# LiuZhu-CV/PAIF

Hardware: AMD Instinct MI355X
Metric: fused image-pairs/sec at 480x640 bs=8 per GPU (fusion-net forward) (higher is better)
Workload: dtype f16 (IEEE fp16 maps and conv weights, one fp16 MFMA per product, f32 accumulate; stems, guided filter and the last map fp32)

## Files before the change

### paif_amd/csrc/conv_dma.h

```cpp
#pragma once
#include <hip/hip_runtime.h>

namespace paif_conv_dma {

struct Args {
  const void* src[3];
  const void* res[3];
  const void* wpk;
  const float* scale;
  const float* shift;
  const float* prelu;
  void* out;
  float alpha;
  int nsrc, nres, act, kh;
  int cout;
  int B, H, W, reverse;
  float* cpool;
  int f16;
  int dil;
  int in_relu;
};

bool eligible(int nsrc, int nres, int B, int H, int W, float alpha);
bool eligible16(int nsrc, int nres, int B, int H, int W, float alpha);
bool eligible7(int nsrc, int nres, int B, int H, int W, float alpha);
bool eligible_d2(int nsrc, int nres, int B, int H, int W, float alpha);
bool can_cpool(int nsrc, int nres, int kh, int cout, int dil);
int launch(const Args& a, hipStream_t st);

bool eligible_1x1(int nsrc, int nres, int B, int H, int W);
int launch_1x1(const Args& a, hipStream_t st);

}
```

### paif_amd/csrc/conv_mfma.hip

```cpp
#include <stdlib.h>

#include "conv_dma.h"
#include "paif_common.h"
#include <type_traits>

#ifndef PAIF_UB_HOOKS
#define PAIF_UB_HOOKS 3
#endif
#ifndef PAIF_UB
#define PAIF_UB 11
#endif

namespace {

typedef float f32x16 __attribute__((ext_vector_type(16)));

#ifndef PAIF_TH
#define PAIF_TH 8
#endif
constexpr int TH = PAIF_TH;
constexpr int TW = 32;
constexpr int NTHREADS = 256;
constexpr int SEGS_PER_WAVE = TH / 4;

// ... 1292 lines not shown
  } else {
    const int t = tid - 4 * 64;
    const int q = t & 7, px = t >> 3;
    const float4 sc = *reinterpret_cast<const float4*>((a.scale ? a.scale : k_ones) + 4 * q);
    const float4 sh = *reinterpret_cast<const float4*>((a.shift ? a.shift : k_zeros) + 4 * q);
    const float slope = *(a.act == 1 ? a.prelu : k_zeros);
    const int nres = a.res[0] ? (a.res[1] ? (a.res[2] ? 3 : 2) : 1) : 0;
    const unsigned lane_off = (unsigned)px * 32u + 4u * (unsigned)q;
    auto run = [&](auto nres_c) {
      constexpr int NR = decltype(nres_c)::value;
      float4 r[NR > 0 ? NR : 1][8];
      auto request = [&](int i) {
        int b, y0, x0;
        tile_of(min(i, cnt - 1), b, y0, x0);
        const size_t base = ((size_t)(b * a.H + y0) * a.W + x0) * 32;
        const unsigned lo = x0 + px < a.W ? lane_off : 0u;
#pragma unroll
        for (int k = 0; k < NR; ++k)
#pragma unroll
          for (int j = 0; j < 8; ++j) {
            const int yy = min(y0 + j, a.H - 1) - y0;
            r[k][j] = paif::ldq_nt<BFR>(a.res[k], base + (size_t)yy * a.W * 32 + lo);
          }
      };
      if (cnt > 0) request(0);
      int s2 = 0, i2 = 0;
      for (int g = 0; g <= S + 1; ++g) {
        if (g >= 2) {
          if (s2 == nsrc - 1) {
            int b, y0, x0;
            tile_of(i2, b, y0, x0);
            float4 o[8];
#pragma unroll
            for (int j = 0; j < 8; ++j) o[j] = *reinterpret_cast<const float4*>(outbuf + (j * 32 + px) * 32 + 4 * q);
            const size_t base = ((size_t)(b * a.H + y0) * a.W + x0) * 32;
            const bool colok = x0 + px < a.W;
#pragma unroll
            for (int j = 0; j < 8; ++j) {
              float4 v = o[j];
              v.x = v.x * sc.x + sh.x; v.y = v.y * sc.y + sh.y; v.z = v.z * sc.z + sh.z; v.w = v.w * sc.w + sh.w;
              if (a.act == 1) {
                v.x = paif::prelu_f(v.x, slope); v.y = paif::prelu_f(v.y, slope);
                v.z = paif::prelu_f(v.z, slope); v.w = paif::prelu_f(v.w, slope);
              } else if (a.act == 2) {
                v.x = fmaxf(v.x, 0.f); v.y = fmaxf(v.y, 0.f); v.z = fmaxf(v.z, 0.f); v.w = fmaxf(v.w, 0.f);
              }
              v.x *= a.alpha; v.y *= a.alpha; v.z *= a.alpha; v.w *= a.alpha;
#pragma unroll
              for (int k = 0; k < NR; ++k) { v.x += r[k][j].x; v.y += r[k][j].y; v.z += r[k][j].z; v.w += r[k][j].w; }
              if (colok && y0 + j < a.H)
                paif::stq_nt<BFO>(a.out, base + (size_t)j * a.W * 32 + lane_off, v);
              if (a.cpool) {
                float mx = fmaxf(fmaxf(v.x, v.y), fmaxf(v.z, v.w)), sm = (v.x + v.y) + (v.z + v.w);
                paif::pix8_max_sum(mx, sm);
                if (colok && y0 + j < a.H && q == 0)
                  *reinterpret_cast<float2*>(a.cpool + ((base + (size_t)j * a.W * 32) >> 5) * 4 + (size_t)px * 4) = make_float2(mx, sm * (1.0f / 32.0f));
              }
            }
            if (NR > 0) request(i2 + 1);
          }
          if (++s2 == nsrc) { s2 = 0; ++i2; }
        }
        lds_barrier();
        lds_barrier();
      }
    };
    if (nres == 0) run(std::integral_constant<int, 0>{});
    else if (nres == 1) run(std::integral_constant<int, 1>{});
    else if (nres == 2) run(std::integral_constant<int, 2>{});
    else run(std::integral_constant<int, 3>{});
  }
}

template <int KH, int DIL, int ST = 0>
__global__ __launch_bounds__(WS_THREADS, 1) void conv_bf16x3_ws(ConvArgs a, int ntiles) { conv_ws_body<KH, DIL, ST, false>(a, ntiles); }
template <int KH, int DIL, int ST = 0>
__global__ __launch_bounds__(WS_THREADS, 1) void conv_bf16x3_wsr(ConvArgs a, int ntiles) { conv_ws_body<KH, DIL, ST, true>(a, ntiles); }

template <int KH, int DIL, int ST = 0>
int launch_bf16x3_ws(const ConvArgs& a, hipStream_t st) {
  constexpr int P = DIL * (KH - 1) / 2;
  constexpr size_t lds_bytes = 2 * (size_t)(TH + 2 * P) * (TW + 2 * P) * 144 + 8 * 32 * 32 * 4;
  static_assert(lds_bytes <= 160 * 1024, "two tile buffers + the parked tile do not fit LDS");
  static bool raised = false;
  constexpr bool HAS_RELU = KH == 3 && DIL == 2 && paif::st_in(ST) != 0 && paif::st_low(ST) != 7;
  if (!raised) {
    hipError_t e = hipFuncSetAttribute(reinterpret_cast<const void*>(&conv_bf16x3_ws<KH, DIL, ST>),
                                       hipFuncAttributeMaxDynamicSharedMemorySize, (int)lds_bytes);
    if constexpr (HAS_RELU) {
      if (e == hipSuccess)
        e = hipFuncSetAttribute(reinterpret_cast<const void*>(&conv_bf16x3_wsr<KH, DIL, ST>), hipFuncAttributeMaxDynamicSharedMemorySize,
                                (int)lds_bytes);
    }
    if (e != hipSuccess) {
      paif::set_error("conv2d(bf16x3 ws): cannot raise dynamic LDS to %zu: %s", lds_bytes, hipGetErrorString(e));
      return (int)e;
    }
    raised = true;
  }
  if (a.in_act == 2) {
    if constexpr (HAS_RELU) {
      hipLaunchKernelGGL((conv_bf16x3_wsr<KH, DIL, ST>), dim3(256), dim3(WS_THREADS), lds_bytes, st, a, a.nblk);
      PAIF_LAUNCH_CHECK("conv2d(bf16x3 wsr)");
      return 0;
    }
    paif::set_error("conv2d(bf16x3 ws): input ReLU is built for the bf16-stored dilation-2 3x3 only");
    return PAIF_ENOSUP;
  }
  hipLaunchKernelGGL((conv_bf16x3_ws<KH, DIL, ST>), dim3(256), dim3(WS_THREADS), lds_bytes, st, a, a.nblk);
  PAIF_LAUNCH_CHECK("conv2d(bf16x3 ws)");
  return 0;
}

static inline bool ws_enabled() {
  static const bool on = [] {
    const char* e = getenv("PAIF_CONV_WS");
    return !(e && e[0] == '0');
  }();
  return on;
}
static inline bool st_h16(const ConvArgs& a) { return a.st == 1 || a.st == 3; }
static inline bool st_is_f16(const ConvArgs& a) { return a.st >= 3; }
static inline bool ws_eligible(const ConvArgs& a) {
  return ws_enabled() && a.nblk >= 1024 && !a.pool_partial && a.cout == 32 && (a.in_act == 0 || (a.in_act == 2 && st_h16(a))) &&
         (size_t)a.H * a.W * 128 < ((size_t)1 << 32);
}

static inline bool res_eligible(const ConvArgs& a) {
  static const bool on = [] {
    const char* e = getenv("PAIF_CONV_RES");
    return !(e && e[0] == '0');
  }();
  static const int ms_res = [] {
    const char* e = getenv("PAIF_CONV_RES_NSRC");
    return e ? atoi(e) : 1;
  }();
  return on && !st_is_f16(a) && (a.nsrc == 1 || (a.wl0 && a.st == 1 && a.in_act == 0 && a.nsrc <= ms_res)) && a.nblk >= 2048 && a.cout == 32 && a.in_act <= 2 && (PAIF_RES_ROWS == 8 || !a.pool_partial) &&
         (size_t)a.B * a.H * a.W * 128 < ((size_t)1 << 31);
}

static inline bool needs_hooks(const ConvArgs& a) { return a.in_act >= 3 || a.aux_out || a.epi_dact; }

static inline bool takes_ws(const ConvArgs& a, int kh, int dil) {
#if PAIF_TH == 8
  if (needs_hooks(a) || kh > 3 || !ws_eligible(a)) return false;
  if (a.st == 4) return dil == 2 && a.nsrc == 1 && a.in_act == 0;
  if (kh == 1) return !a.res[0] && a.in_act == 0;
  return dil == 2 && a.nsrc == 1 && st_h16(a);
#else
  return false;
#endif
}

enum ConvVariant { CV_PLAIN, CV_HOOKS, CV_WS, CV_RES, CV_MS, CV_DMA };
static inline int res_count(const ConvArgs& a) { return a.res[0] ? (a.res[1] ? (a.res[2] ? 3 : 2) : 1) : 0; }
static inline ConvVariant bf16x3_variant(const ConvArgs& a, int kh, int dil) {
  if (needs_hooks(a)) return CV_HOOKS;
  if (dil == 1 && st_h16(a) && a.wl0 && a.in_act == 0 && !a.pool_partial &&
      ((kh == 3 && a.cout == 32 && paif_conv_dma::eligible(a.nsrc, res_count(a), a.B, a.H, a.W, a.alpha)) ||
       (kh == 3 && a.cout == 16 && paif_conv_dma::eligible16(a.nsrc, res_count(a), a.B, a.H, a.W, a.alpha)) ||
       (kh == 7 && a.cout == 32 && paif_conv_dma::eligible7(a.nsrc, res_count(a), a.B, a.H, a.W, a.alpha))))
    return CV_DMA;
  if (kh == 3 && dil == 2 && st_h16(a) && a.wl0 && a.in_act == 2 && !a.pool_partial && a.cout == 32 &&
      paif_conv_dma::eligible_d2(a.nsrc, res_count(a), a.B, a.H, a.W, a.alpha))
    return CV_DMA;
  if (kh == 1 && dil == 1 && st_h16(a) && a.wl0 && a.in_act == 0 && !a.pool_partial && a.cout == 32 && ws_eligible(a) &&
      paif_conv_dma::eligible_1x1(a.nsrc, res_count(a), a.B, a.H, a.W))
    return CV_DMA;
  if (takes_ws(a, kh, dil)) return CV_WS;
  if (kh == 3 && dil == 1 && !st_is_f16(a)) {
    if (res_eligible(a)) return CV_RES;
    if (ms_enabled() && a.nsrc >= 2 && a.cout == 32 && a.in_act == 0 && !a.pool_partial &&
        (size_t)a.B * a.H * a.W * 128 < ((size_t)1 << 32))
      return CV_MS;
  }
  return CV_PLAIN;
}

static inline bool variant_can_cpool(const ConvArgs& a, int kh, int dil) {
  if (a.cout != 32 || needs_hooks(a)) return false;
  if (bf16x3_variant(a, kh, dil) == CV_DMA) return paif_conv_dma::can_cpool(a.nsrc, res_count(a), kh, a.cout, dil);
  return true;
}

template <int KH, int DIL, int ST>
int launch_bf16x3_st(const ConvArgs& a, hipStream_t st) {
  switch (bf16x3_variant(a, KH, DIL)) {
    case CV_DMA: {
      paif_conv_dma::Args d{};
      for (int s = 0; s < 3; ++s) { d.src[s] = a.src[s]; d.res[s] = a.res[s]; }
      d.wpk = a.wpk; d.scale = a.scale; d.shift = a.shift; d.prelu = a.prelu; d.out = a.out; d.alpha = a.alpha;
      d.nsrc = a.nsrc; d.nres = res_count(a); d.act = a.act; d.B = a.B; d.H = a.H; d.W = a.W; d.reverse = a.reverse; d.kh = KH; d.cout = a.cout;
      d.f16 = paif::st_f16(ST) ? 1 : 0;
      d.cpool = a.cpool;
      d.dil = DIL; d.in_relu = a.in_act == 2 ? 1 : 0;
      return paif_conv_dma::launch(d, st);
    }
    case CV_HOOKS:
      if constexpr (ST == 0) return launch_bf16x3_h<KH, DIL, true>(a, st);
      paif::set_error("conv2d: the gradient hooks (in_act >= 3, aux_out, epi_dact) are built for fp32 storage only");
      return PAIF_ENOSUP;
    case CV_WS:
#if PAIF_TH == 8
      if constexpr (KH <= 3) return launch_bf16x3_ws<KH, DIL, ST>(a, st);
#endif
      break;
    case CV_RES:
      if constexpr (KH == 3 && DIL == 1 && !paif::st_f16(ST)) {
        if constexpr (ST == 4) {
          if (a.nsrc == 2) return launch_bf16x3_res<3, 1, 2, ST>(a, st);
          if (a.nsrc == 3) return launch_bf16x3_res<3, 1, 3, ST>(a, st);
        }
        return launch_bf16x3_res<3, 1, 1, ST>(a, st);
      }
      break;
    case CV_MS:
      if constexpr (KH == 3 && DIL == 1 && !paif::st_f16(ST)) return a.nsrc == 2 ? launch_bf16x3_ms<3, 1, 2, ST>(a, st) : launch_bf16x3_ms<3, 1, 3, ST>(a, st);
      break;
    default: break;
  }
  return launch_bf16x3_h<KH, DIL, false, ST>(a, st);
}

static inline int kernel_st(const ConvArgs& a) {
  if (a.st == 4) return 15;
  const int st = a.st == 3 ? 1 : a.st;
  const int base = st == 1 ? (a.in_act == 1 ? 3 : 1) : st;
  const int code = (a.wl0 && base) ? base + 3 : base;
  return a.st >= 3 ? code + 8 : code;
}

template <int KH, int DIL>
int launch_bf16x6(const ConvArgs& a, hipStream_t st) {
  if (a.st != 0) {
    paif::set_error("conv2d: precision bf16x6 is built for fp32-stored maps");
    return PAIF_ENOSUP;
  }
  return needs_hooks(a) ? launch_bf16x3_h<KH, DIL, true, 0, 3>(a, st) : launch_bf16x3_h<KH, DIL, false, 0, 3>(a, st);
}

template <int KH, int DIL>
int launch_f16x3(const ConvArgs& a, hipStream_t st) {
  if (a.st != 0) {
    paif::set_error("conv2d: precision f16x3 is built for fp32-stored maps");
    return PAIF_ENOSUP;
  }
  return needs_hooks(a) ? launch_bf16x3_h<KH, DIL, true, 0, 2, 1>(a, st) : launch_bf16x3_h<KH, DIL, false, 0, 2, 1>(a, st);
}

template <int KH, int DIL>
int launch_bf16x3(const ConvArgs& a, hipStream_t st) {
  const int code = kernel_st(a);
  if (code == 0) return launch_bf16x3_st<KH, DIL, 0>(a, st);
  if constexpr ((KH == 1 || KH == 3 || KH == 7) && (DIL == 1 || (KH == 3 && DIL == 2))) {
    switch (code) {
      case 1: return launch_bf16x3_st<KH, DIL, 1>(a, st);
      case 3: return launch_bf16x3_st<KH, DIL, 3>(a, st);
      case 4: return launch_bf16x3_st<KH, DIL, 4>(a, st);
      case 6: return launch_bf16x3_st<KH, DIL, 6>(a, st);
      default: break;
    }
    if constexpr (KH == 1) {
      if (code == 2) return launch_bf16x3_st<KH, DIL, 2>(a, st);
      if (code == 5) return launch_bf16x3_st<KH, DIL, 5>(a, st);
    }
    switch (code) {
      case 12: return launch_bf16x3_st<KH, DIL, 12>(a, st);
      case 14: return launch_bf16x3_st<KH, DIL, 14>(a, st);
      default: break;
    }
    if constexpr (KH == 1) {
      if (code == 9) return launch_bf16x3_st<KH, DIL, 9>(a, st);
    }
    if constexpr (KH == 3 && DIL == 2) {
      if (code == 15) return launch_bf16x3_st<KH, DIL, 15>(a, st);
    }
  }
  paif::set_error("conv2d: storage %d is not built for the %dx%d dilation-%d kernel", a.st, KH, KH, DIL);
  return PAIF_ENOSUP;
}

__global__ void pack_weight_bf16x3_kernel(const float* __restrict__ w, unsigned short* __restrict__ wpk, int cout, int nsrc,
                                          int kh) {
  const int ntap = kh * kh;
  const int total = nsrc * ntap * 2 * 2 * 64 * 8;
  for (int idx = blockIdx.x * blockDim.x + threadIdx.x; idx < total; idx += gridDim.x * blockDim.x) {
    const int j = idx & 7, lane = (idx >> 3) & 63, part = (idx >> 9) & 1, ks = (idx >> 10) & 1;
    int rest = idx >> 11;
    const int tap = rest % ntap;
    const int s = rest / ntap;
    const int n = lane & 31, hh = lane >> 5;
    const int c = s * 32 + 16 * ks + 8 * hh + j;
    const float v = (n < cout) ? w[((size_t)n * (nsrc * 32) + c) * ntap + tap] : 0.f;
    const __bf16 hi = (__bf16)v;
    const __bf16 out = part == 0 ? hi : (__bf16)(v - (float)hi);
    wpk[idx] = __builtin_bit_cast(unsigned short, out);
  }
}

__global__ void compose_dw_pw_kernel(const float* __restrict__ dw, const float* __restrict__ pw, float* __restrict__ out, int cout,
                                     int cin, int ntap) {
  const int total = cout * cin * ntap;
  for (int idx = blockIdx.x * blockDim.x + threadIdx.x; idx < total; idx += gridDim.x * blockDim.x) {
    const int tap = idx % ntap, ci = (idx / ntap) % cin, co = idx / (ntap * cin);
    out[idx] = pw[co * cin + ci] * dw[ci * ntap + tap];
  }
}

__global__ void compose_pw_conv_kernel(const float* __restrict__ pw, const float* __restrict__ w, float* __restrict__ out, int cout, int cmid,
                                       int cin, int ntap) {
  const int total = cout * cin * ntap;
  for (int idx = blockIdx.x * blockDim.x + threadIdx.x; idx < total; idx += gridDim.x * blockDim.x) {
    const int rest = idx % (cin * ntap), co = idx / (cin * ntap);
    double acc = 0.0;
    for (int m = 0; m < cmid; ++m) acc = fma((double)pw[co * cmid + m], (double)w[(size_t)m * cin * ntap + rest], acc);
    out[idx] = (float)acc;
  }
}

__device__ __forceinline__ unsigned short bf16x6_piece(float v, int part) {
  const __bf16 hi = (__bf16)v;
  const float r1 = v - (float)hi;
  const __bf16 mid = (__bf16)r1;
  const __bf16 out = part == 0 ? hi : (part == 1 ? mid : (__bf16)(r1 - (float)mid));
  return __builtin_bit_cast(unsigned short, out);
}
__global__ void pack_weight_bf16x6_kernel(const float* __restrict__ w, unsigned short* __restrict__ wpk, int cout, int nsrc, int kh) {
  const int ntap = kh * kh;
  const int total = nsrc * ntap * 2 * 3 * 64 * 8;
  for (int idx = blockIdx.x * blockDim.x + threadIdx.x; idx < total; idx += gridDim.x * blockDim.x) {
    const int j = idx & 7, lane = (idx >> 3) & 63;
    int rest = idx >> 9;
    const int part = rest % 3; rest /= 3;
    const int ks = rest & 1; rest >>= 1;
    const int tap = rest % ntap;
    const int s = rest / ntap;
    const int n = lane & 31, hh = lane >> 5;
    const int c = s * 32 + 16 * ks + 8 * hh + j;
    const float v = (n < cout) ? w[((size_t)n * (nsrc * 32) + c) * ntap + tap] : 0.f;
    wpk[idx] = bf16x6_piece(v, part);
  }
}
__global__ void pack_decomp1x1_bf16x6_kernel(const float* __restrict__ w, unsigned short* __restrict__ wpk) {
  const int total = 3 * 2 * 3 * 64 * 8;
  for (int idx = blockIdx.x * blockDim.x + threadIdx.x; idx < total; idx += gridDim.x * blockDim.x) {
    const int j = idx & 7, lane = (idx >> 3) & 63;
    int rest = idx >> 9;
    const int part = rest % 3; rest /= 3;
    const int ks = rest & 1;
// ... 19 lines not shown
    float v;
    if (s == 0) v = wn[64 + c] + wn[96 + c];
    else if (s == 1) v = wn[c] - wn[64 + c];
    else v = wn[32 + c] - wn[96 + c];
    const __bf16 hi = (__bf16)v;
    const __bf16 out = part == 0 ? hi : (__bf16)(v - (float)hi);
    wpk[idx] = __builtin_bit_cast(unsigned short, out);
  }
}

__device__ __forceinline__ unsigned short f16x2_piece(float v, int part) {
  const _Float16 hi = (_Float16)v;
  const _Float16 out = part == 0 ? hi : (_Float16)(v - (float)hi);
  return __builtin_bit_cast(unsigned short, out);
}
__global__ void pack_weight_f16x2_kernel(const float* __restrict__ w, unsigned short* __restrict__ wpk, int cout, int nsrc, int kh) {
  const int ntap = kh * kh;
  const int total = nsrc * ntap * 2 * 2 * 64 * 8;
  for (int idx = blockIdx.x * blockDim.x + threadIdx.x; idx < total; idx += gridDim.x * blockDim.x) {
    const int j = idx & 7, lane = (idx >> 3) & 63, part = (idx >> 9) & 1, ks = (idx >> 10) & 1;
    int rest = idx >> 11;
    const int tap = rest % ntap;
    const int s = rest / ntap;
    const int n = lane & 31, hh = lane >> 5;
    const int c = s * 32 + 16 * ks + 8 * hh + j;
    const float v = (n < cout) ? w[((size_t)n * (nsrc * 32) + c) * ntap + tap] : 0.f;
    wpk[idx] = f16x2_piece(v, part);
  }
}
__global__ void pack_decomp1x1_hf_f16x2_kernel(const float* __restrict__ w, unsigned short* __restrict__ wpk) {
  const int total = 3 * 2 * 2 * 64 * 8;
  for (int idx = blockIdx.x * blockDim.x + threadIdx.x; idx < total; idx += gridDim.x * blockDim.x) {
    const int j = idx & 7, lane = (idx >> 3) & 63, part = (idx >> 9) & 1, ks = (idx >> 10) & 1, s = idx >> 11;
    const int n = lane & 31, hh = lane >> 5;
    const int c = 16 * ks + 8 * hh + j;
    const float* wn = w + n * 128;
    float v;
    if (s == 0) v = wn[c] + wn[32 + c];
    else if (s == 1) v = wn[64 + c] - wn[c];
    else v = wn[96 + c] - wn[32 + c];
    wpk[idx] = f16x2_piece(v, part);
  }
}

template <int KH, int DIL, int CIN, bool HOOKS>
int launch_h(const ConvArgs& a, hipStream_t st) {
  constexpr int P = DIL * (KH - 1) / 2;
  constexpr size_t tile_bytes = (size_t)(TH + 2 * P) * (TW + 2 * P) * (CIN + 4) * 4;
  constexpr size_t epi_bytes = (size_t)TH * 32 * 32 * 4;
  constexpr size_t lds_bytes = tile_bytes > epi_bytes ? tile_bytes : epi_bytes;
  static_assert(lds_bytes <= 160 * 1024, "tile does not fit LDS");
  if (lds_bytes > 64 * 1024) {
    hipError_t e = hipFuncSetAttribute(reinterpret_cast<const void*>(&conv_mfma_f32<KH, DIL, CIN, HOOKS>),
                                       hipFuncAttributeMaxDynamicSharedMemorySize, (int)lds_bytes);
    if (e != hipSuccess) {
      paif::set_error("conv2d: cannot raise dynamic LDS to %zu: %s", lds_bytes, hipGetErrorString(e));
      return (int)e;
    }
  }
  hipLaunchKernelGGL((conv_mfma_f32<KH, DIL, CIN, HOOKS>), dim3(a.nblk), dim3(NTHREADS), lds_bytes, st, a);
  PAIF_LAUNCH_CHECK("conv2d");
  return 0;
}

template <int KH, int DIL, int CIN>
int launch(const ConvArgs& a, hipStream_t st) {
  return needs_hooks(a) ? launch_h<KH, DIL, CIN, true>(a, st) : launch_h<KH, DIL, CIN, false>(a, st);
}

__global__ void pack_weight_kernel(const float* __restrict__ w, float* __restrict__ wpk, int cout, int nsrc, int cin,
                                   int kh) {
  const int ntap = kh * kh, no = cin / 8;
  const int total = nsrc * ntap * no * 256;
  for (int idx = blockIdx.x * blockDim.x + threadIdx.x; idx < total; idx += gridDim.x * blockDim.x) {
    const int i = idx & 3, lane = (idx >> 2) & 63;
    int rest = idx >> 8;
    const int o = rest % no; rest /= no;
    const int tap = rest % ntap;
    const int s = rest / ntap;
    const int n = lane & 31, h = lane >> 5;
    const int c = s * cin + 8 * o + 4 * h + i;
    wpk[idx] = (n < cout) ? w[((size_t)n * (nsrc * cin) + c) * ntap + tap] : 0.f;
  }
}

__global__ void pack_decomp1x1_kernel(const float* __restrict__ w, float* __restrict__ wpk) {
  const int total = 3 * 4 * 256;
  for (int idx = blockIdx.x * blockDim.x + threadIdx.x; idx < total; idx += gridDim.x * blockDim.x) {
    const int i = idx & 3, lane = (idx >> 2) & 63;
    const int o = (idx >> 8) & 3, s = idx >> 10;
    const int n = lane & 31, h = lane >> 5;
    const int c = 8 * o + 4 * h + i;
    const float* wn = w + n * 128;
    float v;
    if (s == 0) v = wn[64 + c] + wn[96 + c];
    else if (s == 1) v = wn[c] - wn[64 + c];
    else v = wn[32 + c] - wn[96 + c];
    wpk[idx] = v;
  }
}

__global__ void bn_fold_kernel(const float* g, const float* bta, const float* mean, const float* var, float eps,
                               float* scale, float* shift, int C) {
  const int c = blockIdx.x * blockDim.x + threadIdx.x;
  if (c < C) {
    const float s = g[c] / sqrtf(var[c] + eps);
    scale[c] = s;
    shift[c] = bta[c] - mean[c] * s;
  }
}

}

extern "C" {

int paif_conv2d_blocks(int B, int H, int W) { return B * ((H + TH - 1) / TH) * ((W + TW - 1) / TW); }

size_t paif_conv_wpk_floats(int nsrc, int cin, int kh) { return (size_t)nsrc * kh * kh * (cin / 8) * 256; }

int paif_conv2d_is_persistent(const paif_conv_desc* d, int B, int H, int W) {
  if (!d || (d->precision != PAIF_CONV_BF16X3 && d->precision != PAIF_CONV_BF16 && d->precision != PAIF_CONV_F16 && d->precision != PAIF_CONV_F16X2) ||
      d->cin != 32 || B <= 0 || H <= 0 || W <= 0)
    return 0;
  ConvArgs a{};
  for (int s = 0; s < 3; ++s) a.res[s] = d->res[s];
  a.pool_partial = d->pool_partial; a.nsrc = d->nsrc; a.in_act = d->in_act; a.cout = d->cout;
  a.aux_out = d->aux_out; a.epi_dact = d->epi_dact; a.st = d->storage;
  a.H = H; a.W = W;
  a.nblk = B * ((W + TW - 1) / TW) * ((H + TH - 1) / TH);
  return takes_ws(a, d->kh, d->dil) ? 1 : 0;
}

int paif_conv2d_can_cpool(const paif_conv_desc* d, int B, int H, int W) {
  if (!d || d->cout != 32 || d->cin != 32 || B <= 0 || H <= 0 || W <= 0 || d->precision == PAIF_CONV_F32 || d->precision == PAIF_CONV_BF16X6 || d->precision == PAIF_CONV_F16X3) return 0;
  ConvArgs a{};
  for (int s = 0; s < 3; ++s) a.res[s] = d->res[s];
  a.pool_partial = d->pool_partial; a.nsrc = d->nsrc; a.in_act = d->in_act; a.cout = d->cout;
  a.aux_out = d->aux_out; a.epi_dact = d->epi_dact;
  a.B = B; a.H = H; a.W = W;
  a.nblk = B * ((W + TW - 1) / TW) * ((H + TH - 1) / TH);
  a.st = d->storage; a.wl0 = (d->precision == PAIF_CONV_BF16 || d->precision == PAIF_CONV_F16) ? 1 : 0; a.alpha = d->alpha;
  return variant_can_cpool(a, d->kh, d->dil) ? 1 : 0;
}

int paif_conv2d_kernel_name(const paif_conv_desc* d, int B, int H, int W, char* buf, int buflen) {
  PAIF_REQUIRE(d && buf && buflen > 0 && B > 0 && H > 0 && W > 0, PAIF_EINVAL, "conv2d_kernel_name: bad arguments");
  ConvArgs a{};
  for (int s = 0; s < 3; ++s) a.res[s] = d->res[s];
  a.pool_partial = d->pool_partial; a.nsrc = d->nsrc; a.in_act = d->in_act; a.cout = d->cout;
  a.aux_out = d->aux_out; a.epi_dact = d->epi_dact;
  a.B = B; a.H = H; a.W = W;
  a.nblk = B * ((W + TW - 1) / TW) * ((H + TH - 1) / TH);
  a.st = d->storage; a.wl0 = (d->precision == PAIF_CONV_BF16 || d->precision == PAIF_CONV_F16) ? 1 : 0; a.alpha = d->alpha;
  const int code = kernel_st(a);
  if (d->precision == PAIF_CONV_BF16X6 && d->cin == 32) {
    snprintf(buf, buflen, "conv_mfma_bf16x6<%d, %d, %s, 0>", d->kh, d->dil, needs_hooks(a) ? "true" : "false");
    return 0;
  }
  if (d->precision == PAIF_CONV_F16X3 && d->cin == 32) {
    snprintf(buf, buflen, "conv_mfma_f16x3<%d, %d, %s, 0>", d->kh, d->dil, needs_hooks(a) ? "true" : "false");
    return 0;
  }
  if (d->precision != PAIF_CONV_BF16X3 && d->precision != PAIF_CONV_BF16 && d->precision != PAIF_CONV_F16 && d->precision != PAIF_CONV_F16X2) {
    snprintf(buf, buflen, "conv_mfma_f32<%d, %d, %d, %s>", d->kh, d->dil, d->cin, needs_hooks(a) ? "true" : "false");
    return 0;
  }
  if (d->cin != 32) {
    snprintf(buf, buflen, "conv_mfma_f32<%d, %d, %d, %s>", d->kh, d->dil, d->cin, needs_hooks(a) ? "true" : "false");
    return 0;
  }
  switch (bf16x3_variant(a, d->kh, d->dil)) {
    case CV_DMA:
      if (d->kh == 7) snprintf(buf, buflen, "conv7x7_h16_dma<%d>", a.st >= 3 ? 2 : 1);
      else if (d->kh == 1) snprintf(buf, buflen, "conv_h16_dma_1x1<%d>", a.st >= 3 ? 2 : 1);
      else snprintf(buf, buflen, "conv3x3_h16_dma<%d, %d, %d, %s, %d, %d>", d->nsrc, res_count(a), a.st >= 3 ? 2 : 1, d->cpool ? "true" : "false",
                    d->dil, d->dil == 2 ? 2 : 0);
      break;
    case CV_WS: snprintf(buf, buflen, "conv_bf16x3_ws%s<%d, %d, %d>", d->in_act == 2 ? "r" : "", d->kh, d->dil, code); break;
    case CV_RES: snprintf(buf, buflen, "conv_bf16x3_res<%d, %d, %d, %d, %d>", d->kh, d->dil, d->nsrc, PAIF_RES_ROWS, code); break;
    case CV_MS: snprintf(buf, buflen, "conv_bf16x3_ms<%d, %d, %d, %d>", d->kh, d->dil, d->nsrc, code); break;
    case CV_HOOKS: snprintf(buf, buflen, "conv_mfma_bf16x3<%d, %d, true, %d>", d->kh, d->dil, code); break;
    default: snprintf(buf, buflen, "conv_mfma_bf16x3<%d, %d, false, %d>", d->kh, d->dil, code); break;
  }
  return 0;
}

int paif_conv2d_fwd(const paif_conv_desc* d, int B, int H, int W, paif_stream_t stream) {
  PAIF_REQUIRE(d && d->out && d->wpk, PAIF_EINVAL, "conv2d: null descriptor/out/wpk");
  PAIF_REQUIRE(d->nsrc >= 1 && d->nsrc <= 3, PAIF_EINVAL, "conv2d: nsrc=%d", d->nsrc);
  for (int s = 0; s < d->nsrc; ++s) PAIF_REQUIRE(d->src[s], PAIF_EINVAL, "conv2d: src[%d] null", s);
  PAIF_REQUIRE(d->cout == 32 || d->cout == 16, PAIF_ENOSUP, "conv2d: cout=%d", d->cout);
  PAIF_REQUIRE(B > 0 && H > 0 && W > 0, PAIF_EINVAL, "conv2d: empty shape %dx%dx%d", B, H, W);
  PAIF_REQUIRE(d->in_act != 1 || d->in_prelu, PAIF_EINVAL, "conv2d: in_act=PReLU without slope");
  PAIF_REQUIRE(d->act != 1 || d->prelu, PAIF_EINVAL, "conv2d: act=PReLU without slope");
  ConvArgs a;
  for (int s = 0; s < 3; ++s) {
    a.src[s] = s < d->nsrc ? d->src[s] : nullptr;
    a.res[s] = d->res[s];
  }
  a.wpk = reinterpret_cast<const float4*>(d->wpk);
  a.in_prelu = d->in_prelu; a.scale = d->scale; a.shift = d->shift; a.prelu = d->prelu;
  a.out = d->out; a.pool_partial = d->pool_partial; a.cpool = d->cpool; a.alpha = d->alpha;
  a.nsrc = d->nsrc; a.in_act = d->in_act; a.act = d->act; a.cout = d->cout;
  a.aux_out = d->aux_out; a.in_aux = d->in_aux; a.in_scale = d->in_scale; a.in_alpha = d->in_alpha;
  a.epi_aux = d->epi_aux; a.epi_dact = d->epi_dact;
  PAIF_REQUIRE(d->in_act >= 0 && d->in_act <= 5, PAIF_EINVAL, "conv2d: in_act=%d", d->in_act);
  PAIF_REQUIRE(!(d->in_act == 3 || d->in_act == 4) || (d->in_aux && d->nsrc == 1), PAIF_EINVAL,
               "conv2d: in_act=%d needs in_aux and a single source", d->in_act);
  PAIF_REQUIRE(d->in_act != 3 || d->in_prelu, PAIF_EINVAL, "conv2d: in_act=3 without slope");
  PAIF_REQUIRE(d->epi_dact >= 0 && d->epi_dact <= 2 && (!d->epi_dact || d->epi_aux), PAIF_EINVAL, "conv2d: epi_dact=%d", d->epi_dact);
  PAIF_REQUIRE(d->epi_dact != 1 || d->prelu, PAIF_EINVAL, "conv2d: epi_dact=PReLU without slope");
  a.B = B; a.H = H; a.W = W;
  a.tilesX = (W + TW - 1) / TW; a.tilesY = (H + TH - 1) / TH; a.nblk = B * a.tilesX * a.tilesY;
  a.reverse = d->reverse_tiles ? 1 : 0;
  a.st = d->storage;
  a.wl0 = (d->precision == PAIF_CONV_BF16 || d->precision == PAIF_CONV_F16) ? 1 : 0;
  PAIF_REQUIRE(d->storage >= 0 && d->storage <= 4, PAIF_EINVAL, "conv2d: storage=%d", d->storage);
  const bool st_bf = d->storage == PAIF_ST_BF16 || d->storage == PAIF_ST_F32_BF16, st_hf = d->storage == PAIF_ST_F16 || d->storage == PAIF_ST_F16_F32;
  PAIF_REQUIRE(!st_bf || ((d->precision == PAIF_CONV_BF16X3 || d->precision == PAIF_CONV_BF16) && d->cin == 32), PAIF_ENOSUP,
               "conv2d: bf16 storage needs the split-bf16 kernels (cin 32)");
  PAIF_REQUIRE(!st_hf || ((d->precision == PAIF_CONV_F16 || d->precision == PAIF_CONV_F16X2) && d->cin == 32), PAIF_ENOSUP,
               "conv2d: fp16 storage takes precision F16 / F16X2 (cin 32)");
  PAIF_REQUIRE(d->precision != PAIF_CONV_BF16 || st_bf, PAIF_ENOSUP, "conv2d: precision bf16 is built for bf16-stored maps only");
  PAIF_REQUIRE((d->precision != PAIF_CONV_F16 && d->precision != PAIF_CONV_F16X2) || st_hf, PAIF_ENOSUP,
               "conv2d: precision fp16 is built for fp16-stored maps only");
  PAIF_REQUIRE(d->storage != PAIF_ST_F16_F32 || d->precision == PAIF_CONV_F16, PAIF_ENOSUP, "conv2d: fp16 in / fp32 out takes plain fp16 weights");
  hipStream_t st = paif::as_stream(stream);
  PAIF_REQUIRE(!d->cpool || paif_conv2d_can_cpool(d, B, H, W), PAIF_ENOSUP, "conv2d: no fused ChannelPool for this descriptor (paif_conv2d_can_cpool)");
  PAIF_REQUIRE(d->cin == 32 || d->cin == 16, PAIF_ENOSUP, "conv2d: cin=%d", d->cin);
  PAIF_REQUIRE(d->precision == PAIF_CONV_F32 || d->precision == PAIF_CONV_BF16X3 || d->precision == PAIF_CONV_BF16 ||
                   d->precision == PAIF_CONV_BF16X6 || d->precision == PAIF_CONV_F16 || d->precision == PAIF_CONV_F16X2 ||
                   d->precision == PAIF_CONV_F16X3, PAIF_EINVAL,
               "conv2d: precision=%d", d->precision);
  PAIF_REQUIRE((d->precision != PAIF_CONV_BF16X6 && d->precision != PAIF_CONV_F16X3) || d->cin == 32, PAIF_ENOSUP, "conv2d: bf16x6 / f16x3 need 32-channel sources");
  const int key = d->kh * 100 + d->dil * 10 + (d->cin == 32 ? 0 : 1);
  if (d->precision == PAIF_CONV_F16X3) {
    switch (key) {
      case 110: return launch_f16x3<1, 1>(a, st);
      case 310: return launch_f16x3<3, 1>(a, st);
      case 320: return launch_f16x3<3, 2>(a, st);
      case 510: return launch_f16x3<5, 1>(a, st);
      case 710: return launch_f16x3<7, 1>(a, st);
      default: break;
    }
    paif::set_error("conv2d(f16x3): kernel %dx%d dil %d cin %d not built", d->kh, d->kh, d->dil, d->cin);
    return PAIF_ENOSUP;
  }
  if (d->precision == PAIF_CONV_BF16X6) {
    switch (key) {
      case 110: return launch_bf16x6<1, 1>(a, st);
      case 310: return launch_bf16x6<3, 1>(a, st);
      case 320: return launch_bf16x6<3, 2>(a, st);
      case 510: return launch_bf16x6<5, 1>(a, st);
      case 710: return launch_bf16x6<7, 1>(a, st);
      default: break;
    }
    paif::set_error("conv2d(bf16x6): kernel %dx%d dil %d cin %d not built", d->kh, d->kh, d->dil, d->cin);
    return PAIF_ENOSUP;
  }
  if (d->precision == PAIF_CONV_BF16X3 || d->precision == PAIF_CONV_BF16 || d->precision == PAIF_CONV_F16 || d->precision == PAIF_CONV_F16X2) {
    switch (key) {
      case 110: return launch_bf16x3<1, 1>(a, st);
      case 310: return launch_bf16x3<3, 1>(a, st);
      case 320: return launch_bf16x3<3, 2>(a, st);
      case 510: return launch_bf16x3<5, 1>(a, st);
      case 520: return launch_bf16x3<5, 2>(a, st);
      case 710: return launch_bf16x3<7, 1>(a, st);
      case 720: return launch_bf16x3<7, 2>(a, st);
      default: break;
    }
    paif::set_error("conv2d(bf16x3): kernel %dx%d dil %d cin %d not built", d->kh, d->kh, d->dil, d->cin);
    return PAIF_ENOSUP;
  }
  switch (key) {
    case 110: return launch<1, 1, 32>(a, st);
    case 310: return launch<3, 1, 32>(a, st);
    case 320: return launch<3, 2, 32>(a, st);
    case 510: return launch<5, 1, 32>(a, st);
    case 520: return launch<5, 2, 32>(a, st);
    case 710: return launch<7, 1, 32>(a, st);
    case 720: return launch<7, 2, 32>(a, st);
    case 311: return launch<3, 1, 16>(a, st);
    default: break;
  }
  paif::set_error("conv2d: kernel %dx%d dil %d cin %d not built", d->kh, d->kh, d->dil, d->cin);
  return PAIF_ENOSUP;
}

int paif_pack_conv_weight_bf16x3(const float* w, float* wpk, int cout, int nsrc, int kh, paif_stream_t stream) {
  PAIF_REQUIRE(w && wpk, PAIF_EINVAL, "pack_conv_weight_bf16x3: null pointer");
  PAIF_REQUIRE(cout >= 1 && cout <= 32 && nsrc >= 1 && nsrc <= 3 && kh >= 1 && kh <= 7, PAIF_ENOSUP,
               "pack_conv_weight_bf16x3: cout=%d nsrc=%d kh=%d", cout, nsrc, kh);
  const int total = nsrc * kh * kh * 2048;
  hipLaunchKernelGGL(pack_weight_bf16x3_kernel, dim3((total + 255) / 256), dim3(256), 0, paif::as_stream(stream), w,
                     reinterpret_cast<unsigned short*>(wpk), cout, nsrc, kh);
  PAIF_LAUNCH_CHECK("pack_conv_weight_bf16x3");
  return 0;
}

int paif_pack_conv_weight_f16x2(const float* w, float* wpk, int cout, int nsrc, int kh, paif_stream_t stream) {
  PAIF_REQUIRE(w && wpk, PAIF_EINVAL, "pack_conv_weight_f16x2: null pointer");
  PAIF_REQUIRE(cout >= 1 && cout <= 32 && nsrc >= 1 && nsrc <= 3 && kh >= 1 && kh <= 7, PAIF_ENOSUP,
               "pack_conv_weight_f16x2: cout=%d nsrc=%d kh=%d", cout, nsrc, kh);
  const int total = nsrc * kh * kh * 2048;
  hipLaunchKernelGGL(pack_weight_f16x2_kernel, dim3((total + 255) / 256), dim3(256), 0, paif::as_stream(stream), w,
                     reinterpret_cast<unsigned short*>(wpk), cout, nsrc, kh);
  PAIF_LAUNCH_CHECK("pack_conv_weight_f16x2");
  return 0;
}

int paif_pack_decomp1x1_hf_weight_f16x2(const float* w, float* wpk, paif_stream_t stream) {
  PAIF_REQUIRE(w && wpk, PAIF_EINVAL, "pack_decomp1x1_hf_weight_f16x2: null pointer");
  hipLaunchKernelGGL(pack_decomp1x1_hf_f16x2_kernel, dim3(24), dim3(256), 0, paif::as_stream(stream), w,
                     reinterpret_cast<unsigned short*>(wpk));
  PAIF_LAUNCH_CHECK("pack_decomp1x1_hf_weight_f16x2");
  return 0;
}

int paif_pack_conv_weight_bf16x6(const float* w, float* wpk, int cout, int nsrc, int kh, paif_stream_t stream) {
  PAIF_REQUIRE(w && wpk, PAIF_EINVAL, "pack_conv_weight_bf16x6: null pointer");
  PAIF_REQUIRE(cout >= 1 && cout <= 32 && nsrc >= 1 && nsrc <= 3 && kh >= 1 && kh <= 7, PAIF_ENOSUP,
               "pack_conv_weight_bf16x6: cout=%d nsrc=%d kh=%d", cout, nsrc, kh);
  const int total = nsrc * kh * kh * 3072;
  hipLaunchKernelGGL(pack_weight_bf16x6_kernel, dim3((total + 255) / 256), dim3(256), 0, paif::as_stream(stream), w,
                     reinterpret_cast<unsigned short*>(wpk), cout, nsrc, kh);
  PAIF_LAUNCH_CHECK("pack_conv_weight_bf16x6");
  return 0;
}

int paif_compose_dw_pw_weight(const float* dw, const float* pw, float* out, int cout, int cin, int kh, paif_stream_t stream) {
// ... 60 lines not shown
```

Baseline: 2507.

## Add row-streaming DMA kernel for dilated 3x3 h16 convolutions

Adds a new kernel for 3x3 dilation-2 convolutions with one source and 0-3 residual maps. It is a persistent per-wave row walker. Each wave handles a 32-wide column strip and walks same-parity rows. Input rows are fetched with a multi-slot buffer-to-LDS DMA ring, and weights stay in registers. Residual loads are prefetched a step ahead and an fp32 output variant is added. The goal is to cut the halo re-reads and load latency of tiled dilated convs, but it adds a large amount of hand-scheduled asm with waitcnt assumptions that could be fragile. Eligibility depends on problem size, which 480x640 bs=8 likely meets.

Result: faster. 2539, median of 6 (+1.3%).

```diff
diff --git a/paif_amd/csrc/conv_dma.h b/paif_amd/csrc/conv_dma.h
--- a/paif_amd/csrc/conv_dma.h
+++ b/paif_amd/csrc/conv_dma.h
@@ -19,6 +19,7 @@
   int f16;
   int dil;
   int in_relu;
+  int out_f32;
 };
 
 bool eligible(int nsrc, int nres, int B, int H, int W, float alpha);
@@ -31,4 +32,7 @@
 bool eligible_1x1(int nsrc, int nres, int B, int H, int W);
 int launch_1x1(const Args& a, hipStream_t st);
 
+bool eligible_rows(int nsrc, int nres, int in_relu, int cpool, int f16, int out_f32, int B, int H, int W);
+int launch_rows(const Args& a, hipStream_t st);
+
 }
diff --git a/paif_amd/csrc/conv_dma_rows.hip b/paif_amd/csrc/conv_dma_rows.hip
--- /dev/null
+++ b/paif_amd/csrc/conv_dma_rows.hip
@@ -0,0 +1,340 @@
+#include <stdint.h>
+#include <stdlib.h>
+
+#include <type_traits>
+
+#include "conv_dma.h"
+#include "paif_common.h"
+
+namespace paif_conv_dma {
+namespace {
+
+typedef float f32x16 __attribute__((ext_vector_type(16)));
+typedef unsigned u32x4 __attribute__((ext_vector_type(4)));
+
+constexpr int RW = 32;
+constexpr int RWH = RW + 4;
+constexpr int DPS = 3;
+constexpr int SLOT = DPS * 1024;
+constexpr int NSLOT = 5, PF = NSLOT - 3;
+constexpr int PARK = 32 * 32 * 4;
+constexpr int WAVE_LDS = NSLOT * SLOT + PARK;
+constexpr int WAVES = 4;
+constexpr int LDS_BYTES = WAVES * WAVE_LDS;
+constexpr int MAX_WAVES = 2048;
+constexpr int MIN_RUN = 16;
+static_assert(2 * LDS_BYTES <= 160 * 1024, "two workgroups per CU do not fit LDS");
+static_assert(RWH * 4 <= DPS * 64, "DMA instructions do not cover the row piece");
+constexpr unsigned RSRC_W3 = 0x00020000u;
+constexpr unsigned OOB = 0x80000000u;
+
+#ifndef CR_LD_AUX
+#define CR_LD_AUX 2
+#endif
+#ifndef CR_ST_AUX
+#define CR_ST_AUX 0
+#endif
+#define CR_VMWAIT(n) asm volatile("s_waitcnt vmcnt(%0)" ::"n"(n) : "memory")
+#define CR_RD128(dst, addr, off) asm volatile("ds_read_b128 %0, %1 offset:%2" : "=v"(dst) : "v"(addr), "n"(off) : "memory")
+#define CR_WR32(addr, val, off) asm volatile("ds_write_b32 %0, %1 offset:%2" ::"v"(addr), "v"(val), "n"(off) : "memory")
+
+__device__ __forceinline__ void dma16(__amdgpu_buffer_rsrc_t rsrc, unsigned voff, unsigned lds_off) {
+  __builtin_amdgcn_raw_ptr_buffer_load_lds(rsrc, (__attribute__((address_space(3))) void*)(uintptr_t)lds_off, 16, voff, 0, 0, CR_LD_AUX);
+}
+
+template <int F, int NRES, bool O32>
+__global__ __launch_bounds__(WAVES * 64, 2) void conv3x3_h16_dma_rows(Args a, int total, int SX, int run) {
+  constexpr int D = NRES == 3 ? 1 : 2, NSETS = D + 1, RL = 2 * NRES;
+  constexpr int N_ROW = PF * (RL + DPS);
+  constexpr int N_RES = DPS + D * (RL + DPS);
+  static_assert(N_ROW <= 63 && N_RES <= 63, "vmcnt is 6 bits");
+  __shared__ __attribute__((aligned(16))) unsigned char smem[LDS_BYTES];
+  asm volatile("" ::"v"((unsigned)(uintptr_t)(__attribute__((address_space(3))) unsigned char*)smem) : "memory");
+
+  const int tid = threadIdx.x, l = tid & 63;
+  const int w = __builtin_amdgcn_readfirstlane(tid >> 6);
+  const int p = l & 31, hh = l >> 5;
+  const int gw = blockIdx.x * WAVES + w;
+  int pos = gw * run;
+  const int end = min(total, pos + run);
+  if (pos >= end) return;
+  const int H = a.H, W = a.W;
+  const int n_even = (H + 1) >> 1;
+
+  constexpr int OPITCH = O32 ? 128 : 64;
+  const int map_bytes = a.B * H * W * 64;
+  const __amdgpu_buffer_rsrc_t rs_src = __builtin_amdgcn_make_buffer_rsrc(const_cast<void*>(a.src[0]), 0, map_bytes, RSRC_W3);
+  __amdgpu_buffer_rsrc_t rs_res[NRES > 0 ? NRES : 1];
+#pragma unroll
+  for (int r = 0; r < NRES; ++r) rs_res[r] = __builtin_amdgcn_make_buffer_rsrc(const_cast<void*>(a.res[r]), 0, map_bytes, RSRC_W3);
+  const __amdgpu_buffer_rsrc_t rs_out = __builtin_amdgcn_make_buffer_rsrc(a.out, 0, a.B * H * W * OPITCH, RSRC_W3);
+
+  u32x4 bw[9][2];
+  {
+    const __amdgpu_buffer_rsrc_t rs_w = __builtin_amdgcn_make_buffer_rsrc(const_cast<void*>(a.wpk), 0, 9 * 2 * 2 * 1024, RSRC_W3);
+#pragma unroll
+    for (int tap = 0; tap < 9; ++tap)
+#pragma unroll
+      for (int ks = 0; ks < 2; ++ks) bw[tap][ks] = __builtin_amdgcn_raw_buffer_load_b128(rs_w, (unsigned)l * 16u, ((tap * 2 + ks) * 2) * 1024, 0);
+  }
+  float esc[8], esh[8];
+#pragma unroll
+  for (int j = 0; j < 8; ++j) {
+    const int c = 8 * (l & 3) + j;
+    esc[j] = a.scale ? a.scale[c] : 1.f;
+    esh[j] = a.shift ? a.shift[c] : 0.f;
+  }
+  const bool relu = a.act == 2;
+  const float slope = a.act == 1 ? *a.prelu : 1.f;
+  const float alpha = a.alpha;
+
+  int d_col[DPS];
+  unsigned d_rel[DPS];
+#pragma unroll
+  for (int i = 0; i < DPS; ++i) {
+    const int n = 64 * i + l, c = n >> 2;
+    d_col[i] = c;
+    d_rel[i] = (unsigned)(c * 64 + (((n & 3) ^ ((c >> 2) & 3)) * 16));
+  }
+  const unsigned lds_w = (unsigned)(w * WAVE_LDS);
+  unsigned a_rd[3][2];
+#pragma unroll
+  for (int dx = 0; dx < 3; ++dx)
+#pragma unroll
+    for (int ks = 0; ks < 2; ++ks) {
+      const int c = p + 2 * dx;
+      a_rd[dx][ks] = lds_w + (unsigned)(c * 64 + (((2 * ks + hh) ^ ((c >> 2) & 3)) * 16));
+    }
+  const unsigned a_pw = lds_w + NSLOT * SLOT + (unsigned)((4 * hh * 32 + p) * 4);
+  const unsigned a_pr = lds_w + NSLOT * SLOT + (unsigned)((l >> 2) * 128 + (l & 3) * 32);
+  const unsigned e_lane = (unsigned)l * 16u;
+  const unsigned o_lane = O32 ? (unsigned)((l >> 2) * 128 + (l & 3) * 32) : e_lane;
+
+  u32x4 rr[NSETS][NRES > 0 ? NRES : 1][2];
+  f32x16 acc;
+
+  while (pos < end) {
+    const int q = pos / H, rem = pos - q * H;
+    const int par = rem >= n_even ? 1 : 0;
+    const int i0 = rem - par * n_even;
+    const int nch = par ? H - n_even : n_even;
+    const int n = min(nch - i0, end - pos);
+    const int b = q / SX, x0 = (q - b * SX) * RW;
+    pos += n;
+    bool colok[DPS];
+#pragma unroll
+    for (int i = 0; i < DPS; ++i) colok[i] = d_col[i] < RWH && (unsigned)(x0 - 2 + d_col[i]) < (unsigned)W;
+    const bool xok0 = x0 + (l >> 2) < W, xok1 = x0 + 16 + (l >> 2) < W;
+    auto issue_row = [&](int m, int slot) {
+      const int j = i0 - 1 + m;
+      const unsigned dead = (j >= 0 && j < nch && m <= n + 1) ? 0u : OOB;
+      const unsigned rowb = (unsigned)((b * H + 2 * j + par) * W + x0 - 2) * 64u;
+#pragma unroll
+      for (int i = 0; i < DPS; ++i) dma16(rs_src, (colok[i] ? rowb + d_rel[i] : OOB) | dead, lds_w + (unsigned)(slot * SLOT + i * 1024));
+    };
+    auto issue_res = [&](auto settag, int t) {
+      constexpr int SET = decltype(settag)::value;
+      const bool live = t >= 0 && t < n;
+      const unsigned rowb = (unsigned)((b * H + 2 * (i0 + t) + par) * W + x0) * 64u;
+#pragma unroll
+      for (int r = 0; r < NRES; ++r) {
+        rr[SET][r][0] = __builtin_amdgcn_raw_buffer_load_b128(rs_res[r], (live && xok0) ? rowb + e_lane : OOB, 0, CR_LD_AUX);
+        rr[SET][r][1] = __builtin_amdgcn_raw_buffer_load_b128(rs_res[r], (live && xok1) ? rowb + 1024u + e_lane : OOB, 0, CR_LD_AUX);
+      }
+    };
+    auto issue_step = [&](auto settag, int s, int slot) {
+      if constexpr (NRES > 0) issue_res(settag, s + D);
+      asm volatile("" ::: "memory");
+      issue_row(s + 2 + PF, slot);
+    };
+
+    int cur = 0;
+    auto step = [&](auto settag, int t) {
+      constexpr int SET = decltype(settag)::value;
+      const int s1 = cur + 1 >= NSLOT ? cur + 1 - NSLOT : cur + 1, s2 = cur + 2 >= NSLOT ? cur + 2 - NSLOT : cur + 2;
+      const int fill = cur == 0 ? NSLOT - 1 : cur - 1;
+      issue_step(std::integral_constant<int, (SET + D) % NSETS>{}, t, fill);
+      CR_VMWAIT(N_ROW);
+      const unsigned rb[3] = {(unsigned)(cur * SLOT), (unsigned)(s1 * SLOT), (unsigned)(s2 * SLOT)};
+      u32x4 A[2][3][2];
+      auto read = [&](int buf, int dy) {
+#pragma unroll
+        for (int dx = 0; dx < 3; ++dx)
+#pragma unroll
+          for (int ks = 0; ks < 2; ++ks) {
+            const unsigned ad = a_rd[dx][ks] + rb[dy];
+            CR_RD128(A[buf][dx][ks], ad, 0);
+          }
+      };
+      auto mma = [&](auto dytag) {
+        constexpr int dy = decltype(dytag)::value, buf = dy & 1;
+#pragma unroll
+        for (int dx = 0; dx < 3; ++dx)
+#pragma unroll
+          for (int ks = 0; ks < 2; ++ks) {
+            if (dy == 0 && dx == 0 && ks == 0) {
+              const f32x16 z = {0.f, 0.f, 0.f, 0.f, 0.f, 0.f, 0.f, 0.f, 0.f, 0.f, 0.f, 0.f, 0.f, 0.f, 0.f, 0.f};
+              acc = paif::mfma16<F>(A[buf][dx][ks], bw[dy * 3 + dx][ks], z);
+            } else {
+              acc = paif::mfma16<F>(A[buf][dx][ks], bw[dy * 3 + dx][ks], acc);
+            }
+          }
+      };
+      read(0, 0);
+      read(1, 1);
+      asm volatile("s_waitcnt lgkmcnt(6)"
+                   : "+v"(A[0][0][0]), "+v"(A[0][0][1]), "+v"(A[0][1][0]), "+v"(A[0][1][1]), "+v"(A[0][2][0]), "+v"(A[0][2][1])::"memory");
+      __builtin_amdgcn_sched_barrier(0);
+      mma(std::integral_constant<int, 0>{});
+      __builtin_amdgcn_sched_barrier(0);
+      read(0, 2);
+      asm volatile("s_waitcnt lgkmcnt(6)"
+                   : "+v"(A[1][0][0]), "+v"(A[1][0][1]), "+v"(A[1][1][0]), "+v"(A[1][1][1]), "+v"(A[1][2][0]), "+v"(A[1][2][1])::"memory");
+      __builtin_amdgcn_sched_barrier(0);
+      mma(std::integral_constant<int, 1>{});
+      __builtin_amdgcn_sched_barrier(0);
+      asm volatile("s_waitcnt lgkmcnt(0)"
+                   : "+v"(A[0][0][0]), "+v"(A[0][0][1]), "+v"(A[0][1][0]), "+v"(A[0][1][1]), "+v"(A[0][2][0]), "+v"(A[0][2][1])::"memory");
+      __builtin_amdgcn_sched_barrier(0);
+      mma(std::integral_constant<int, 2>{});
+      __builtin_amdgcn_sched_barrier(0);
+
+      asm volatile("s_nop 15\n\ts_nop 7" ::: "memory");
+#pragma unroll
+      for (int r = 0; r < 16; ++r) {
+        const float v = acc[r];
+        CR_WR32(a_pw, v, ((r & 3) + 8 * (r >> 2)) * 128);
+      }
+      u32x4 tq[2][2];
+      CR_RD128(tq[0][0], a_pr, 0);
+      CR_RD128(tq[0][1], a_pr, 16);
+      CR_RD128(tq[1][0], a_pr, 2048);
+      CR_RD128(tq[1][1], a_pr, 2048 + 16);
+      asm volatile("s_waitcnt lgkmcnt(0)" : "+v"(tq[0][0]), "+v"(tq[0][1]), "+v"(tq[1][0]), "+v"(tq[1][1])::"memory");
+      if constexpr (NRES > 0 && N_RES < N_ROW) {
+        CR_VMWAIT(N_RES);
+      }
+      __builtin_amdgcn_sched_barrier(0);
+      const unsigned orow = (unsigned)((b * H + 2 * (i0 + t) + par) * W + x0) * (unsigned)OPITCH;
+#pragma unroll
+      for (int it = 0; it < 2; ++it) {
+        float ev[8];
+#pragma unroll
+        for (int j = 0; j < 8; ++j) {
+          float v = __builtin_fmaf(__uint_as_float(tq[it][j >> 2][j & 3]), esc[j], esh[j]);
+          const float vp = paif::prelu_f(v, slope), vr = fmaxf(v, 0.f);
+          v = relu ? vr : vp;
+          if constexpr (NRES == 0) {
+            v = v * alpha;
+          } else {
+#pragma unroll
+            for (int r = 0; r < NRES; ++r) {
+              const unsigned u = rr[SET][r][it][j >> 1];
+              float rv;
+              if constexpr (F == 2) rv = (float)__builtin_bit_cast(paif::f16x2_t, u)[j & 1];
+              else rv = __uint_as_float((j & 1) ? (u & 0xffff0000u) : (u << 16));
+              v = r == 0 ? __builtin_fmaf(v, alpha, rv) : v + rv;
+            }
+          }
+          ev[j] = v;
+        }
+        const bool ok = it ? xok1 : xok0;
+        if constexpr (O32) {
+          u32x4 o0 = {__float_as_uint(ev[0]), __float_as_uint(ev[1]), __float_as_uint(ev[2]), __float_as_uint(ev[3])};
+          u32x4 o1 = {__float_as_uint(ev[4]), __float_as_uint(ev[5]), __float_as_uint(ev[6]), __float_as_uint(ev[7])};
+          const unsigned off = ok ? orow + (unsigned)(it * 16 * OPITCH) + o_lane : OOB;
+          __builtin_amdgcn_raw_buffer_store_b128(o0, rs_out, off, 0, CR_ST_AUX);
+          asm volatile("s_nop 2" : "+v"(o0));
+          __builtin_amdgcn_raw_buffer_store_b128(o1, rs_out, ok ? off + 16u : OOB, 0, CR_ST_AUX);
+          asm volatile("s_nop 2" : "+v"(o1));
+        } else {
+          const uint2 h0 = paif::f32_to_h4<F>(make_float4(ev[0], ev[1], ev[2], ev[3]));
+          const uint2 h1 = paif::f32_to_h4<F>(make_float4(ev[4], ev[5], ev[6], ev[7]));
+          u32x4 od = {h0.x, h0.y, h1.x, h1.y};
+          __builtin_amdgcn_raw_buffer_store_b128(od, rs_out, ok ? orow + (unsigned)(it * 16 * OPITCH) + o_lane : OOB, 0, CR_ST_AUX);
+          asm volatile("s_nop 2" : "+v"(od));
+        }
+      }
+      __builtin_amdgcn_sched_barrier(0);
+      cur = s1;
+    };
+
+    static_assert(PF == 2, "the prologue lists 2 + PF = 4 virtual steps");
+    auto vstep = [&](auto stag) {
+      constexpr int S = decltype(stag)::value;
+      issue_step(std::integral_constant<int, (((S + D) % NSETS) + NSETS) % NSETS>{}, S, S + 2 + PF);
+    };
+    vstep(std::integral_constant<int, -4>{});
+    vstep(std::integral_constant<int, -3>{});
+    vstep(std::integral_constant<int, -2>{});
+    vstep(std::integral_constant<int, -1>{});
+    for (int t = 0;; t += NSETS) {
+      step(std::integral_constant<int, 0>{}, t);
+      if (t + 1 >= n) break;
+      step(std::integral_constant<int, 1 % NSETS>{}, t + 1);
+      if (t + 2 >= n) break;
+      if constexpr (NSETS > 2) {
+        step(std::integral_constant<int, 2 % NSETS>{}, t + 2);
+        if (t + 3 >= n) break;
+      }
+    }
+    CR_VMWAIT(0);
+  }
+}
+
+int env_rows() {
+  const char* d = getenv("PAIF_CONV_DMA");
+  if (d && d[0] == '0') return 0;
+  const char* e = getenv("PAIF_CONV_DMA_ROWS");
+  if (!e || !e[0]) return -1;
+  return e[0] == '0' ? 0 : 1;
+}
+
+template <int F, int NRES, bool O32>
+void launch_rows_f(const Args& a, hipStream_t st) {
+  const int SX = (a.W + RW - 1) / RW;
+  const int total = a.B * SX * a.H;
+  const int per = (total + MAX_WAVES - 1) / MAX_WAVES;
+  const int run = per > MIN_RUN ? per : MIN_RUN;
+  const int waves = (total + run - 1) / run;
+  hipLaunchKernelGGL((conv3x3_h16_dma_rows<F, NRES, O32>), dim3((waves + WAVES - 1) / WAVES), dim3(WAVES * 64), 0, st, a, total, SX, run);
+}
+
+}
+
+bool eligible_rows(int nsrc, int nres, int in_relu, int cpool, int f16, int out_f32, int B, int H, int W) {
+  const int sw = env_rows();
+  if (sw == 0 || nsrc != 1 || nres < 0 || nres > 3 || in_relu || cpool || (out_f32 && !f16)) return false;
+  if ((long long)B * H * W * (out_f32 ? 128 : 64) >= (1ll << 31)) return false;
+  if (sw == 1) return true;
+  return H >= 64 && (long long)B * H * ((W + RW - 1) / RW) >= (long long)MIN_RUN * MAX_WAVES;
+}
+
+int launch_rows(const Args& a, hipStream_t st) {
+  if (a.nsrc != 1 || a.cout != 32 || a.cpool || a.in_relu || a.dil != 2 || a.kh != 3 || a.nres < 0 || a.nres > 3 || (a.out_f32 && !a.f16)) {
+    paif::set_error("conv2d(h16 dma rows): built for one source, dilation 2, 0-3 residual maps, no input activation, no ChannelPool");
+    return PAIF_ENOSUP;
+  }
+#define CR_LAUNCH(NR)                                                              \
+  case NR:                                                                         \
+    if (a.out_f32) launch_rows_f<2, NR, true>(a, st);                              \
+    else if (a.f16) launch_rows_f<2, NR, false>(a, st);                            \
+    else launch_rows_f<1, NR, false>(a, st);                                       \
+    break;
+  switch (a.nres) {
+    CR_LAUNCH(0)
+    CR_LAUNCH(1)
+    CR_LAUNCH(2)
+    CR_LAUNCH(3)
+    default: break;
+  }
+#undef CR_LAUNCH
+  hipError_t e = hipGetLastError();
+  if (e != hipSuccess) {
+    paif::set_error("conv2d(h16 dma rows): launch failed: %s", hipGetErrorString(e));
+    return (int)e;
+  }
+  return 0;
+}
+
+}
diff --git a/paif_amd/csrc/conv_mfma.hip b/paif_amd/csrc/conv_mfma.hip
--- a/paif_amd/csrc/conv_mfma.hip
+++ b/paif_amd/csrc/conv_mfma.hip
@@ -1468,7 +1468,7 @@
 #endif
 }
 
-enum ConvVariant { CV_PLAIN, CV_HOOKS, CV_WS, CV_RES, CV_MS, CV_DMA };
+enum ConvVariant { CV_PLAIN, CV_HOOKS, CV_WS, CV_RES, CV_MS, CV_DMA, CV_ROWS };
 static inline int res_count(const ConvArgs& a) { return a.res[0] ? (a.res[1] ? (a.res[2] ? 3 : 2) : 1) : 0; }
 static inline ConvVariant bf16x3_variant(const ConvArgs& a, int kh, int dil) {
   if (needs_hooks(a)) return CV_HOOKS;
@@ -1477,6 +1477,9 @@
        (kh == 3 && a.cout == 16 && paif_conv_dma::eligible16(a.nsrc, res_count(a), a.B, a.H, a.W, a.alpha)) ||
        (kh == 7 && a.cout == 32 && paif_conv_dma::eligible7(a.nsrc, res_count(a), a.B, a.H, a.W, a.alpha))))
     return CV_DMA;
+  if (kh == 3 && dil == 2 && (st_h16(a) || a.st == 4) && a.wl0 && a.in_act == 0 && !a.pool_partial && !a.cpool && a.cout == 32 &&
+      paif_conv_dma::eligible_rows(a.nsrc, res_count(a), 0, 0, st_is_f16(a) ? 1 : 0, a.st == 4 ? 1 : 0, a.B, a.H, a.W))
+    return CV_ROWS;
   if (kh == 3 && dil == 2 && st_h16(a) && a.wl0 && a.in_act == 2 && !a.pool_partial && a.cout == 32 &&
       paif_conv_dma::eligible_d2(a.nsrc, res_count(a), a.B, a.H, a.W, a.alpha))
     return CV_DMA;
@@ -1501,7 +1504,9 @@
 
 template <int KH, int DIL, int ST>
 int launch_bf16x3_st(const ConvArgs& a, hipStream_t st) {
-  switch (bf16x3_variant(a, KH, DIL)) {
+  const ConvVariant cv = bf16x3_variant(a, KH, DIL);
+  switch (cv) {
+    case CV_ROWS:
     case CV_DMA: {
       paif_conv_dma::Args d{};
       for (int s = 0; s < 3; ++s) { d.src[s] = a.src[s]; d.res[s] = a.res[s]; }
@@ -1510,7 +1515,8 @@
       d.f16 = paif::st_f16(ST) ? 1 : 0;
       d.cpool = a.cpool;
       d.dil = DIL; d.in_relu = a.in_act == 2 ? 1 : 0;
-      return paif_conv_dma::launch(d, st);
+      d.out_f32 = paif::st_out(ST) == 0 ? 1 : 0;
+      return cv == CV_ROWS ? paif_conv_dma::launch_rows(d, st) : paif_conv_dma::launch(d, st);
     }
     case CV_HOOKS:
       if constexpr (ST == 0) return launch_bf16x3_h<KH, DIL, true>(a, st);
@@ -1836,6 +1842,7 @@
   a.B = B; a.H = H; a.W = W;
   a.nblk = B * ((W + TW - 1) / TW) * ((H + TH - 1) / TH);
   a.st = d->storage; a.wl0 = (d->precision == PAIF_CONV_BF16 || d->precision == PAIF_CONV_F16) ? 1 : 0; a.alpha = d->alpha;
+  a.cpool = d->cpool;
   const int code = kernel_st(a);
   if (d->precision == PAIF_CONV_BF16X6 && d->cin == 32) {
     snprintf(buf, buflen, "conv_mfma_bf16x6<%d, %d, %s, 0>", d->kh, d->dil, needs_hooks(a) ? "true" : "false");
@@ -1860,6 +1867,7 @@
       else snprintf(buf, buflen, "conv3x3_h16_dma<%d, %d, %d, %s, %d, %d>", d->nsrc, res_count(a), a.st >= 3 ? 2 : 1, d->cpool ? "true" : "false",
                     d->dil, d->dil == 2 ? 2 : 0);
       break;
+    case CV_ROWS: snprintf(buf, buflen, "conv3x3_h16_dma_rows<%d, %d, %s>", a.st >= 3 ? 2 : 1, res_count(a), a.st == 4 ? "true" : "false"); break;
     case CV_WS: snprintf(buf, buflen, "conv_bf16x3_ws%s<%d, %d, %d>", d->in_act == 2 ? "r" : "", d->kh, d->dil, code); break;
     case CV_RES: snprintf(buf, buflen, "conv_bf16x3_res<%d, %d, %d, %d, %d>", d->kh, d->dil, d->nsrc, PAIF_RES_ROWS, code); break;
     case CV_MS: snprintf(buf, buflen, "conv_bf16x3_ms<%d, %d, %d, %d>", d->kh, d->dil, d->nsrc, code); break;
```
